# mikeoliphant/NeuralAudio

Hardware: AMD Instinct MI355X
Metric: concurrent 48 kHz real-time streams + Msamples/s/GPU, NAM WaveNet Standard (higher is better)
Workload: dtype f32 (f16x3-split MFMA, f32 accumulate)

## Files before the change

### neuralaudio_amd/csrc/wavenet_spec_impl.h

```cpp
#pragma once

#include <algorithm>
#include <atomic>
#include <cstddef>
#include <cstdlib>

#include <hip/hip_runtime.h>

#include "device_once.h"
#include <cstring>
#include <type_traits>
#include <vector>

#include "tuning.h"
#include "wavenet_split_dev.h"

namespace na
{
	namespace spk
	{
		using namespace sp;

#ifndef NA_SPK_NT_DIL
#define NA_SPK_NT_DIL 256
#endif
#ifndef NA_SPK_NT_LD
#define NA_SPK_NT_LD 0
#endif
#ifndef NA_SPK_NT_ST
#define NA_SPK_NT_ST 0
#endif
#ifndef NA_SPK_DELAY
#define NA_SPK_DELAY 0
#endif
#ifndef NA_SPK_AUX2
#define NA_SPK_AUX2 0
#endif
		typedef __attribute__((address_space(3))) char* LdsPtr;
		__device__ __forceinline__ u32x4 LdsRead16(unsigned addr) { return *reinterpret_cast<__attribute__((address_space(3))) const u32x4*>((LdsPtr)(size_t)addr); }
		__device__ __forceinline__ u32x2 LdsRead8(unsigned addr) { return *reinterpret_cast<__attribute__((address_space(3))) const u32x2*>((LdsPtr)(size_t)addr); }
		__device__ __forceinline__ void LdsWrite16(unsigned addr, u32x4 v) { *reinterpret_cast<__attribute__((address_space(3))) u32x4*>((LdsPtr)(size_t)addr) = v; }

		template <bool COH>
		__device__ __forceinline__ float LoadIn(const float* p)
		{
			if constexpr (COH) return __builtin_bit_cast(float, __hip_atomic_load(reinterpret_cast<const unsigned*>(p), __ATOMIC_RELAXED, __HIP_MEMORY_SCOPE_SYSTEM));
			else return *p;
		}
		template <bool COH>
		__device__ __forceinline__ void StoreOut(float* p, float v)
		{
			if constexpr (COH) __hip_atomic_store(reinterpret_cast<unsigned*>(p), __builtin_bit_cast(unsigned, v), __ATOMIC_RELAXED, __HIP_MEMORY_SCOPE_SYSTEM);
			else *p = v;
		}

		struct ArchA1Base
		{
			static constexpr int K(int, int) { return 3; }
			static constexpr int HEADK = 1;
			static constexpr bool LEAKY = false;
			static constexpr int T = 2, CHUNK = 10;
			static constexpr bool COARSE = false;
			static constexpr bool GUARDHIST = false;
			static constexpr bool FOLD = false;
			static constexpr int SKEW = 0;
			static constexpr bool COMPACT = true;
#ifndef NA_A1_NT_DIL
#define NA_A1_NT_DIL 128
#endif
			static constexpr int NT_DIL = NA_A1_NT_DIL;
		};
#ifndef NA_SPK_SKEW
#define NA_SPK_SKEW 0
#endif
		struct ArchStd : ArchA1Base
		{
			static constexpr int SKEW = NA_SPK_SKEW;
			static constexpr bool FOLD = true;
			static constexpr int NA = 2;
			static constexpr int CH[2] = { 16, 8 };
			static constexpr int NLA[2] = { 10, 10 };
			static constexpr int DIL[2][16] = { { 1, 2, 4, 8, 16, 32, 64, 128, 256, 512 }, { 1, 2, 4, 8, 16, 32, 64, 128, 256, 512 } };
		};
		struct ArchLite : ArchA1Base
		{
			static constexpr int NA = 2;
			static constexpr int CH[2] = { 16, 8 };
			static constexpr int NLA[2] = { 7, 13 };
			static constexpr int DIL[2][16] = { { 1, 2, 4, 8, 16, 32, 64 }, { 128, 256, 512, 1, 2, 4, 8, 16, 32, 64, 128, 256, 512 } };
		};
		struct ArchLite16 : ArchA1Base
		{
			static constexpr int NA = 2;
			static constexpr int CH[2] = { 16, 16 };
			static constexpr int NLA[2] = { 7, 13 };
			static constexpr int DIL[2][16] = { { 1, 2, 4, 8, 16, 32, 64 }, { 128, 256, 512, 1, 2, 4, 8, 16, 32, 64, 128, 256, 512 } };
		};

		struct ArchLite16T1 : ArchLite16 { static constexpr int T = 1; };

		struct ArchA2Base
		{
			static constexpr int NA = 1;
			static constexpr int NLA[2] = { 23, 0 };
			static constexpr int DIL[2][32] = { { 1, 3, 7, 17, 41, 101, 239, 1, 3, 7, 17, 41, 101, 239, 1, 13, 1, 3, 7, 17, 41, 101, 239 }, { 0 } };
			static constexpr int K(int, int l) { return (l == 14 || l == 15) ? 15 : 6; }
			static constexpr int HEADK = 16;
			static constexpr bool LEAKY = true;
			static constexpr int CHUNK = 16;
			static constexpr bool COARSE = true;
			static constexpr bool GUARDHIST = true;
			static constexpr bool FOLD = false;
			static constexpr int SKEW = 0;
			static constexpr bool COMPACT = false;
			static constexpr int NT_DIL = 100;
		};
		struct ArchA2Full : ArchA2Base { static constexpr int CH[2] = { 8, 0 }; static constexpr int T = 2; };
		struct ArchA2Lite : ArchA2Base { static constexpr int CH[2] = { 4, 0 }; static constexpr int T = 4; };

		struct FamStd { typedef ArchStd A0; typedef ArchStd A1; static constexpr int N = 1; };
		struct FamLite { typedef ArchLite A0; typedef ArchLite A1; static constexpr int N = 1; };
		struct FamLitePacked { typedef ArchLite A0; typedef ArchLite16 A1; static constexpr int N = 2; };
		struct FamA2 { typedef ArchA2Full A0; typedef ArchA2Lite A1; static constexpr int N = 2; };
		struct FamLite16T1 { typedef ArchLite16T1 A0; typedef ArchLite16T1 A1; static constexpr int N = 1; };

		enum TapClass { TAP_LDS = 0, TAP_HIST = 1, TAP_BOTH = 2 };

		template <class A>
		struct Tab
		{
			static constexpr int NA = A::NA;
			static constexpr int TotalLayers() { int n = 0; for (int a = 0; a < NA; a++) n += A::NLA[a]; return n; }
			static constexpr int NL = TotalLayers();
			static constexpr int NSTAGES = NL + NA + 1;
			static constexpr int ArrOf(int L) { int a = 0; while (L >= A::NLA[a]) { L -= A::NLA[a]; a++; } return a; }
			static constexpr int InArr(int L) { int a = 0; while (L >= A::NLA[a]) { L -= A::NLA[a]; a++; } return L; }
			static constexpr int Dil(int L) { return A::DIL[ArrOf(L)][InArr(L)]; }
			static constexpr int GPof(int a) { return A::CH[a] / 4; }
			static constexpr bool FirstOfArr(int L) { return InArr(L) == 0; }
			static constexpr bool LastOfArr(int L) { return InArr(L) == A::NLA[ArrOf(L)] - 1; }
			static constexpr int KS(int L) { return A::K(ArrOf(L), InArr(L)); }
			static constexpr bool Fold(int L) { return A::FOLD && KS(L) == 3 && GPof(ArrOf(L)) >= 2; }
			static constexpr int HEADK = A::HEADK;
			static constexpr int NRINGS = NL + (HEADK > 1 ? 1 : 0);
			static constexpr bool ExactRing(int L) { return L < NL && !FirstOfArr(L) && Dil(L) >= FRAMES && (KS(L) - 1) * Dil(L) >= 2 * FRAMES && ((KS(L) - 1) * Dil(L)) % 16 == 0; }
			static constexpr int HistFrames(int L) { return L < NL ? ((KS(L) - 1) * Dil(L) + 15) / 16 * 16 : (HEADK - 1 + 15) / 16 * 16; }
			static constexpr bool CompactRing(int L) { return A::COMPACT && L < NL && KS(L) > 1 && HistFrames(L) <= WN_COMPACT_MAX_HISTORY; }
			static constexpr int RingFrames(int L)
			{
				if (ExactRing(L)) return (KS(L) - 1) * Dil(L);
				if (CompactRing(L)) return 3 * HistFrames(L);
				return HistFrames(L) + FRAMES;
			}
			static constexpr int RingKeep(int L) { return ExactRing(L) ? RingFrames(L) : (CompactRing(L) ? HistFrames(L) : RingFrames(L) - FRAMES); }
			static constexpr int RingG(int L) { return GPof(L < NL ? ArrOf(L) : NA - 1); }
			static constexpr int RingOff(int L)
			{
				int o = WN_HEADER_F4;
				for (int l = 0; l < L; l++) o += RingFrames(l) * RingG(l);
				return o;
			}
			static constexpr int StateF4 = (RingOff(NRINGS) + 15) / 16 * 16;
			static constexpr int StageOfLayer(int L) { return 1 + L + ArrOf(L); }
			static constexpr int FirstLayerOfArr(int a) { int L = 0; for (int i = 0; i < a; i++) L += A::NLA[i]; return L; }
			static constexpr int LinkStage(int a) { return FirstLayerOfArr(a) + a; }
			static constexpr int LinkNC(int a) { const int Po = 4 / GPof(a - 1), Pn = 4 / GPof(a); return Po > Pn ? Po : Pn; }
			static constexpr int LayerOfStage(int s)
			{
				for (int L = 0; L < NL; L++)
					if (StageOfLayer(L) == s) return L;
				return -1;
			}
			static constexpr int StageOps(int s)
			{
				if (s == 0) return 1;
				if (s == NSTAGES - 1) return 2 * HEADK + 1;
				for (int a = 1; a < NA; a++)
					if (s == LinkStage(a)) return 4 * LinkNC(a) + 1;
				return 2 * KS(LayerOfStage(s)) + 4;
			}
			static constexpr int AOff(int s) { int o = 0; for (int i = 0; i < s; i++) o += StageOps(i) * 64; return o; }
			static constexpr int WsplitQuads = AOff(NSTAGES);
			static constexpr int CHUNK = A::CHUNK;
			static constexpr int TapOps(int s) { return s == NSTAGES - 1 ? 2 * HEADK : 2 * KS(LayerOfStage(s)); }
			static constexpr bool Chunked(int s) { return StageOps(s) > CHUNK; }
			static constexpr int TapChunks(int s) { return (TapOps(s) + CHUNK - 1) / CHUNK; }
			static constexpr int NumChunks(int s) { return Chunked(s) ? TapChunks(s) + 1 : 1; }
			static constexpr int ChunkBegin(int s, int c)
			{
				if (!Chunked(s)) return 0;
				if (c >= TapChunks(s)) return TapOps(s);
				const int pairs = TapOps(s) / 2, n = TapChunks(s);
				return 2 * ((pairs * c + n - 1) / n);
			}
			static constexpr int ChunkEnd(int s, int c) { return !Chunked(s) ? StageOps(s) : (c >= TapChunks(s) ? StageOps(s) : ChunkBegin(s, c + 1)); }
			static constexpr int ChunkIndex(int s, int c) { int n = 0; for (int i = 0; i < s; i++) n += NumChunks(i); return n + c; }
			static constexpr int MaxChunkOps()
			{
				int m = 0;
				for (int s = 0; s < NSTAGES; s++)
					for (int c = 0; c < NumChunks(s); c++) m = (ChunkEnd(s, c) - ChunkBegin(s, c)) > m ? (ChunkEnd(s, c) - ChunkBegin(s, c)) : m;
				return m;
			}
			static constexpr int MaxGP() { int m = 0; for (int a = 0; a < NA; a++) m = GPof(a) > m ? GPof(a) : m; return m; }
		};

		template <class A_, int NF_, int SPB_, bool PK_, bool COH_ = false, bool NT_ = false>
		struct Cfg
		{
			static constexpr bool COH = COH_;
			static constexpr bool NT = NT_;
			typedef A_ A;
			typedef Tab<A_> TB;
			static constexpr int NF = NF_, T = A_::T, FW = 16 * T, WPS = NF_ / FW, SPB = SPB_ * T / 2, NTHREADS = 64 * WPS * SPB;
			static_assert(WPS >= 1 && WPS * FW == NF_, "block length is a whole number of waves");
			static constexpr bool PK = PK_;
			static constexpr int MAXOPS = A_::CHUNK;
			static_assert(TB::MaxChunkOps() <= MAXOPS, "stage operand chunk");
			static constexpr int HPF = 5;
			static constexpr int SKEW = (SPB == 2 && !PK_ && T == 2 && A_::SKEW > 0) ? A_::SKEW : 0;
			static constexpr int NWB = SKEW > 0 ? SPB : 1;
			static constexpr int STG_THREADS = NTHREADS / NWB;
			static constexpr bool AUX16 = !PK_ && SKEW == 0;
			static constexpr int AUX_OFF = 0;
			static constexpr int IMG_OFF = AUX_OFF + SPB * FRAMES * (PK_ ? 32 : (AUX16 ? 16 : 8));
			static constexpr int IMG_ONE = TB::MaxGP() * PLANE * 16;
			static constexpr int WBUF_OFF = IMG_OFF + SPB * 2 * IMG_ONE;
			static constexpr int WBUF_ONE = MAXOPS * 1024;
			static constexpr int IDOP_OFF = WBUF_OFF + NWB * 2 * WBUF_ONE;
			static constexpr int DUMP_OFF = IDOP_OFF + 1024;
			static constexpr int FLAG_OFF = DUMP_OFF + 1024;
			static constexpr int BCAST_OFF = FLAG_OFF + 16 * SPB;
			static constexpr int LDS_BYTES = BCAST_OFF + (COH_ ? 64 : 0);
			static_assert(LDS_BYTES <= 80 * 1024, "two workgroups per CU");
		};

		template <int GP, int T>
		struct Geo
		{
			static_assert(GP == 4 || GP == 2 || GP == 1, "full lane modes of 16 / 8 / 4 channels");
			static constexpr int P = 4 / GP;
			static_assert(T % P == 0, "every tile slot of a set is a tile of the wave");
			static constexpr int S = T / P;
		};

		constexpr int TapClassOf(int F0, int P, int i, int shift)
		{
			const int lo = F0 + 16 * P * i - shift, hi = lo + 16 * P - 1;
			return hi < 0 ? TAP_HIST : (lo >= 0 ? TAP_LDS : TAP_BOTH);
		}

		template <class C, int RG>
		constexpr bool SmallRing() { return C::A::GUARDHIST && C::TB::RingKeep(RG) <= GUARD; }

		template <class C>
		constexpr int WaveTapClass(int w, int P, int i, int shift, bool small)
		{
			if (small) return TAP_LDS;
			if (!C::A::COARSE || w == 0 || C::WPS <= 2) return TapClassOf(C::FW * w, P, i, shift);
			const int first = TapClassOf(C::FW * 1, P, i, shift);
			for (int v = 2; v < C::WPS; v++)
				if (TapClassOf(C::FW * v, P, i, shift) != first) return TAP_BOTH;
			return first;
		}

		template <class C, int L>
		struct LayerSig
		{
			typedef typename C::TB TB;
			static constexpr int GP = TB::GPof(TB::ArrOf(L)), P = Geo<GP, C::T>::P, S = Geo<GP, C::T>::S, d = TB::Dil(L), K = TB::KS(L);
			static constexpr bool NEXT = !TB::LastOfArr(L);
			static constexpr int LN = NEXT ? L + 1 : L;
			static constexpr int dn = NEXT ? TB::Dil(LN) : 0, Kn = NEXT ? TB::KS(LN) : 1;
			static constexpr bool FOLD = TB::Fold(L) && !C::PK;
			static constexpr unsigned long long Of(int w)
			{
				unsigned long long s = 0;
				for (int k = 0; k < K - 1; k++)
					for (int i = 0; i < S; i++) s = s * 3 + (unsigned)WaveTapClass<C>(w, P, i, d * (K - 1 - k), SmallRing<C, L>());
				for (int k = 0; k < Kn - 1 && k < C::HPF; k++)
					for (int i = 0; i < S; i++) s = s * 3 + (unsigned)WaveTapClass<C>(w, P, i, dn * (Kn - 1 - k), SmallRing<C, LN>());
				return s;
			}
			static constexpr int Rep(int w) { int r = w; for (int v = w - 1; v >= 0; v--) if (Of(v) == Of(w)) r = v; return r; }
			static constexpr unsigned MaskOf(int r) { unsigned m = 0; for (int w = 0; w < C::WPS; w++) if (Rep(w) == r) m |= 1u << w; return m; }
			static constexpr bool LastRep(int r) { for (int w = r + 1; w < C::WPS; w++) if (Rep(w) == w) return false; return true; }
		};

		struct Ctx
		{
			__amdgpu_buffer_rsrc_t srsrc;
			__amdgpu_buffer_rsrc_t wrsrc;
			int myPos;
			int wave, sub, waveAll;
			int lane;
			int gs0, gs1;
			unsigned wbuf;
			int stgWave;
#ifdef NA_SP_TRACE
			long long* trace;
			int nwaves;
#endif
		};

#ifdef NA_SP_TRACE
#define SPK_STAMP(stage, point) do { __builtin_amdgcn_sched_barrier(0); if (cx.trace != nullptr && cx.lane == 0) cx.trace[(((stage) * 8 + (point)) * cx.nwaves) + cx.waveAll] = (long long)__builtin_readcyclecounter(); __builtin_amdgcn_sched_barrier(0); } while (0)
#else
#define SPK_STAMP(stage, point) (void)0
#endif

		template <class C, int GP>
		struct Lanes
// ... 127 lines not shown
			return (C::NF - C::FW) + 16 * P * (i + 1) - 1 >= C::NF - KEEP;
		}
		template <class C, int RG>
		constexpr int StoresOf()
		{
			constexpr int S = Geo<C::TB::RingG(RG), C::T>::S;
			int n = 0;
			for (int i = 0; i < S; i++) n += StoreNeeded<C, RG>(i) ? 1 : 0;
			return n;
		}

		template <class C, int RG, int GP, int MINSHIFT>
		__device__ __forceinline__ void Publish(const Ctx& cx, const Lanes<C, GP>& ln, u32x4 v, int i, int imgWrite)
		{
			typedef typename C::TB TB;
			constexpr int P = Geo<GP, C::T>::P, R = TB::RingFrames(RG), OFF = TB::RingOff(RG), KEEP = TB::RingKeep(RG);
			static_assert(GP == TB::RingG(RG), "lane mode of the receiving ring");
			if (!(NA_ABL & 64) && MINSHIFT < C::NF)
				LdsWrite16(ln.img + (unsigned)(imgWrite * C::IMG_ONE + 16 * P * i * 16), v);
			if ((NA_ABL & 4) || !StoreNeeded<C, RG>(i)) return;
			const int pos0 = __builtin_amdgcn_readlane(cx.myPos, RG);
			int base;
			if constexpr (TB::CompactRing(RG))
			{
				int end = pos0 + C::NF % R;
				if (end >= R) end -= R;
				base = end - C::NF + C::FW * cx.wave + 16 * P * i + R;
			}
			else
			{
				base = pos0 + C::FW * cx.wave + 16 * P * i;
				if (base >= R) base -= R;
			}
			const int addr = RingWrap<GP, R>(ln.ring, base);
			constexpr int NT_ST = C::NT ? 2 : NA_SPK_NT_ST, NT_DIL = C::NT ? C::A::NT_DIL : NA_SPK_NT_DIL;
			constexpr bool LONG = RG < TB::NL && TB::Dil(RG < TB::NL ? RG : 0) >= NT_DIL;
			if constexpr (LONG && NT_ST != 0)
			{
				if (KEEP >= C::NF) RingStoreAux<NT_ST>(cx.srsrc, v, addr, OFF * 16);
				else RingStoreAux<NT_ST>(cx.srsrc, v, (C::FW * cx.wave + 16 * P * i + ln.fl >= C::NF - KEEP) ? addr : OOB, OFF * 16);
				return;
			}
			if (KEEP >= C::NF) RingStore(cx.srsrc, v, addr, OFF * 16);
			else RingStore(cx.srsrc, v, (C::FW * cx.wave + 16 * P * i + ln.fl >= C::NF - KEEP) ? addr : OOB, OFF * 16);
		}

		template <class C, int RG, int GP>
		__device__ __forceinline__ void GuardStage(const Ctx& cx, const Lanes<C, GP>& ln, int imgBuf)
		{
			typedef typename C::TB TB;
			static_assert(GP == TB::RingG(RG), "lane mode of the ring");
			constexpr int R = TB::RingFrames(RG), OFF = TB::RingOff(RG);
			if constexpr (!C::A::GUARDHIST) return;
			if (cx.wave != 0) return;
			if constexpr (SmallRing<C, RG>())
			{
				if (NA_ABL & 4) return;
				const int pos0 = __builtin_amdgcn_readlane(cx.myPos, RG);
				int base = pos0 - GUARD;
				if (base < 0) base += R;
				if (cx.lane < 16)
				{
#pragma unroll
					for (int cg = 0; cg < GP; cg++)
					{
						const int addr = RingWrap<GP, R>((unsigned)((cx.lane * GP + cg) * 16), base);
						const unsigned dst = (unsigned)(C::IMG_OFF + imgBuf * C::IMG_ONE + cg * PLANE * 16) + (unsigned)(cx.sub * 2 * C::IMG_ONE);
						__builtin_amdgcn_raw_ptr_buffer_load_lds(cx.srsrc, (__attribute__((address_space(3))) void*)(LdsPtr)(size_t)dst, 16, addr, OFF * 16, 0, 0);
					}
				}
			}
			else
			{
				if ((cx.lane >> 4) < GP && (cx.lane & 15) == 15) LdsWrite16(ln.img + (unsigned)(imgBuf * C::IMG_ONE) - 16u * 16u, u32x4{ 0, 0, 0, 0 });
			}
		}

		template <class C, int SN, int CN>
		struct Stager
		{
			typedef typename C::TB TB;
			static constexpr int QUADS = (TB::ChunkEnd(SN, CN) - TB::ChunkBegin(SN, CN)) * 64;
			static constexpr int SRC = TB::AOff(SN) + TB::ChunkBegin(SN, CN) * 64;
			static constexpr int BUF = TB::ChunkIndex(SN, CN) & 1;
			static constexpr int NCOPY = (QUADS + C::STG_THREADS - 1) / C::STG_THREADS;
			static __device__ __forceinline__ void Begin(const Ctx& cx)
			{
				if (NA_ABL & 16) return;
#pragma unroll
				for (int c = 0; c < NCOPY; c++)
				{
					const int i0 = c * C::STG_THREADS + cx.stgWave * 64;
					const bool mine = i0 < QUADS;
					const unsigned dst = mine ? cx.wbuf + (unsigned)(BUF * C::WBUF_ONE) + (unsigned)i0 * 16u : (unsigned)C::DUMP_OFF;
					__builtin_amdgcn_raw_ptr_buffer_load_lds(cx.wrsrc, (__attribute__((address_space(3))) void*)(LdsPtr)(size_t)dst, 16,
						mine ? (SRC + i0 + cx.lane) * 16 : OOB, 0, 0, 0);
				}
			}
			template <int LATER>
			static __device__ __forceinline__ void End()
			{
				__builtin_amdgcn_s_waitcnt((LATER & 15) | ((LATER >> 4) << 14) | (7 << 4) | (15 << 8));
			}
		};
		template <class C, int s, int c>
		struct NextChunk
		{
			static constexpr bool SAME = c + 1 < C::TB::NumChunks(s);
			static constexpr int S = SAME ? s : s + 1, CN = SAME ? c + 1 : 0;
			typedef Stager<C, S, CN> St;
		};

		template <class C>
		__device__ __forceinline__ u32x4 WOp(const Ctx& cx, int s, int c, int m)
		{
			const int buf = C::TB::ChunkIndex(s, c) & 1, local = m - C::TB::ChunkBegin(s, c);
			return LdsRead16(cx.wbuf + (unsigned)(buf * C::WBUF_ONE + ((NA_ABL & 128) ? 0 : local) * 1024) + (unsigned)cx.lane * 16u);
		}

		template <bool PACKED>
		__device__ __forceinline__ f32x4 ActivateTanh(f32x4 a)
		{
			if (PACKED)
			{
				const f32x2 lo = FastTanh2(f32x2{ a.x, a.y }), hi = FastTanh2(f32x2{ a.z, a.w });
				return f32x4{ lo.x, lo.y, hi.x, hi.y };
			}
			return f32x4{ FastTanh(a.x), FastTanh(a.y), FastTanh(a.z), FastTanh(a.w) };
		}

		template <class C, int GP>
		__device__ __forceinline__ u32x4 TapLds(const Ctx& cx, const Lanes<C, GP>& ln, int imgRead, int shift, int i, int cls)
		{
			constexpr int P = Geo<GP, C::T>::P;
			if (NA_ABL & 256) return u32x4{ (unsigned)shift, 0, 0, 0 };
			if (cls == TAP_LDS) return LdsRead16(ln.img + (unsigned)(imgRead * C::IMG_ONE) + (unsigned)((16 * P * i - shift) * 16));
			int off = C::FW * cx.wave + 16 * P * i + ln.fl - shift;
			off = off < -1 ? -1 : off;
			return LdsRead16((unsigned)(C::IMG_OFF + imgRead * C::IMG_ONE + GUARD * 16) + (unsigned)(cx.sub * 2 * C::IMG_ONE) + (unsigned)((ln.cg * PLANE + off) * 16));
		}

		template <class C, int RG, int GP, int WR>
		__device__ __forceinline__ f32x4 ConvTap(const Ctx& cx, const Lanes<C, GP>& ln, int imgRead, int shift, int i, u32x4 ah, u32x4 al, u32x4 hist, f32x4 acc)
		{
			constexpr int P = Geo<GP, C::T>::P;
			const int cls = WaveTapClass<C>(WR, P, i, shift, SmallRing<C, RG>());
			if (cls != TAP_LDS)
			{
				acc = Mfma(ah, hist, acc);
				acc = MfmaLo<1>(al, hist, acc);
			}
			if (cls != TAP_HIST)
			{
				const u32x4 b = TapLds<C, GP>(cx, ln, imgRead, shift, i, cls);
				acc = Mfma(ah, b, acc);
				acc = MfmaLo<1>(al, b, acc);
			}
			return acc;
		}

		template <class C, int RG, int GP, int WR>
		__device__ __forceinline__ f32x4 ConvTapFold(const Ctx& cx, const Lanes<C, GP>& ln, int imgRead, int shift, int i, u32x4 ah, u32x4 hist, f32x4 acc, u32x2& th)
		{
			constexpr int P = Geo<GP, C::T>::P;
			const int cls = WaveTapClass<C>(WR, P, i, shift, SmallRing<C, RG>());
			th = u32x2{ 0, 0 };
			if (cls != TAP_LDS)
			{
				acc = Mfma(ah, hist, acc);
				th = u32x2{ hist.x, hist.y };
			}
			if (cls != TAP_HIST)
			{
				const u32x4 b = TapLds<C, GP>(cx, ln, imgRead, shift, i, cls);
				acc = Mfma(ah, b, acc);
				th = cls == TAP_LDS ? u32x2{ b.x, b.y } : u32x2{ th.x | b.x, th.y | b.y };
			}
			return acc;
		}

		template <class C, int L, int WR, int c>
		__device__ __forceinline__ void LayerChunk(const Ctx& cx, const Lanes<C, C::TB::GPof(C::TB::ArrOf(L))>& ln, State& st, u32x4 (&ax)[LayerSig<C, L>::S],
			f32x4 (&acc)[LayerSig<C, L>::S])
		{
			typedef typename C::TB TB;
			typedef LayerSig<C, L> SG;
			constexpr int GP = SG::GP, S = SG::S, K = SG::K, s = TB::StageOfLayer(L), NCH = TB::NumChunks(s), CB = TB::ChunkBegin(s, c), CE = TB::ChunkEnd(s, c);
			constexpr int imgRead = s & 1, imgWrite = (s + 1) & 1, LN = SG::LN;
			constexpr bool LASTLAYER = TB::LastOfArr(L) && TB::ArrOf(L) == TB::NA - 1;
			constexpr int NEXTMINSHIFT = SG::NEXT ? TB::Dil(LN) : (1 << 20);
			constexpr bool OWN = 2 * (K - 1) >= CB && 2 * (K - 1) < CE;
			constexpr bool TAIL = 2 * K >= CB && 2 * K < CE;
			constexpr int LATER = ((OWN && SG::NEXT) ? HistLoadsOf<C, LN>() : 0) + ((TAIL && SG::NEXT && !LASTLAYER) ? StoresOf<C, LN>() : 0);
			typedef typename NextChunk<C, s, c>::St NextStager;
			if constexpr (c == 0)
			{
				if constexpr (SG::NEXT) GuardStage<C, LN, GP>(cx, ln, imgWrite);
				else if constexpr (LASTLAYER && TB::HEADK > 1) GuardStage<C, TB::NL, GP>(cx, ln, (TB::NSTAGES - 1 + 1) & 1);
			}
			NextStager::Begin(cx);
			if constexpr (c == 0)
			{
#pragma unroll
				for (int i = 0; i < S; i++) ax[i] = AuxRead<C, GP>(ln, i);
			}
			constexpr int KLO = CB / 2, KHI = (CE / 2 < K - 1) ? CE / 2 : K - 1;
			constexpr int NX = (KHI > C::HPF) ? KHI - (KLO > C::HPF ? KLO : C::HPF) : 0;
			u32x4 hx[NX > 0 ? NX : 1][S];
#pragma unroll
			for (int k = KLO; k < KHI; k++)
			{
				if (k < C::HPF) continue;
#pragma unroll
				for (int i = 0; i < S; i++)
					if (WaveTapClass<C>(WR, SG::P, i, ShiftOf<C, L>(k), SmallRing<C, L>()) != TAP_LDS) hx[k - (KLO > C::HPF ? KLO : C::HPF)][i] = HistLoadAt<C, L, WR>(cx, ln.ring, ln.fl, ShiftOf<C, L>(k), i);
			}
			static_assert(!SG::FOLD || (NCH == 1 && K == 3), "folded operands: K = 3 layers in one chunk");
			u32x2 th[SG::FOLD ? 2 : 1][S];
#pragma unroll
			for (int k = KLO; k < KHI; k++)
			{
				const u32x4 ah = WOp<C>(cx, s, c, 2 * k), al = SG::FOLD ? ah : WOp<C>(cx, s, c, 2 * k + 1);
#pragma unroll
				for (int i = 0; i < S; i++)
				{
					u32x4 h = u32x4{ 0, 0, 0, 0 };
					if (WaveTapClass<C>(WR, SG::P, i, ShiftOf<C, L>(k), SmallRing<C, L>()) != TAP_LDS)
						h = (k < C::HPF) ? st.hist[k < C::HPF ? k : 0][i] : hx[k >= C::HPF ? k - (KLO > C::HPF ? KLO : C::HPF) : 0][i];
					if constexpr (SG::FOLD) acc[i] = ConvTapFold<C, L, GP, WR>(cx, ln, imgRead, ShiftOf<C, L>(k), i, ah, h, acc[i], th[k < 2 ? k : 0][i]);
					else acc[i] = ConvTap<C, L, GP, WR>(cx, ln, imgRead, ShiftOf<C, L>(k), i, ah, al, h, acc[i]);
				}
			}
			if constexpr (SG::FOLD)
			{
				const u32x4 al01 = WOp<C>(cx, s, c, 1);
#pragma unroll
				for (int i = 0; i < S; i++) acc[i] = Mfma(al01, u32x4{ th[0][i].x, th[0][i].y, th[1][i].x, th[1][i].y }, acc[i]);
			}
			if constexpr (OWN)
			{
				if constexpr (SG::NEXT) HistPrefetch<C, LN, WR>(cx, ln.ring, ln.fl, st);
				const u32x4 ah = WOp<C>(cx, s, c, 2 * K - 2), al = WOp<C>(cx, s, c, 2 * K - 1);
#pragma unroll
				for (int i = 0; i < S; i++)
				{
					acc[i] = Mfma(ah, st.xs[i], acc[i]);
					if constexpr (SG::FOLD) acc[i] = Mfma(al, u32x4{ st.xs[i].x, st.xs[i].y, ax[i].x, ax[i].y }, acc[i]);
					else acc[i] = MfmaLo<1>(al, st.xs[i], acc[i]);
				}
			}
			if constexpr (TAIL)
			{
				if constexpr (!SG::FOLD)
				{
					const u32x4 xa = WOp<C>(cx, s, c, 2 * K);
#pragma unroll
					for (int i = 0; i < S; i++) acc[i] = Mfma(xa, ax[i], acc[i]);
				}
				SPK_STAMP(s, 1);
				f32x4 z[S];
#pragma unroll
				for (int i = 0; i < S; i++)
				{
					if constexpr (C::A::LEAKY) z[i] = f32x4{ LeakyReLU(acc[i].x), LeakyReLU(acc[i].y), LeakyReLU(acc[i].z), LeakyReLU(acc[i].w) };
					else z[i] = ActivateTanh<(NA_PK_TANH != 0) && (C::NTHREADS < 512)>(acc[i]);
				}
				SPK_STAMP(s, 2);
				const u32x4 idop = LdsRead16((unsigned)C::IDOP_OFF + (unsigned)cx.lane * 16u);
				const u32x4 w1h = WOp<C>(cx, s, c, 2 * K + 1), w1l = WOp<C>(cx, s, c, 2 * K + 2), b1a = SG::FOLD ? w1l : WOp<C>(cx, s, c, 2 * K + 3);
#pragma unroll
				for (int i = 0; i < S; i++)
				{
					const u32x4 zs = SplitQuad(z[i]);
					st.hd[i] = Mfma(idop, zs, st.hd[i]);
					if constexpr (!LASTLAYER)
					{
						f32x4 y = st.xc[i];
						y = Mfma(w1h, zs, y);
						const u32x4 axi = NA_SPK_AUX2 ? AuxRead<C, GP>(ln, i) : ax[i];
						if constexpr (SG::FOLD) y = Mfma(w1l, u32x4{ zs.x, zs.y, axi.x, axi.y }, y);
						else
						{
							y = MfmaLo<2>(w1l, zs, y);
							y = Mfma(b1a, axi, y);
						}
						st.xc[i] = y;
						if constexpr (SG::NEXT)
						{
							st.xs[i] = Split<C>(y, cx);
							Publish<C, LN, GP, NEXTMINSHIFT>(cx, ln, st.xs[i], i, imgWrite);
						}
					}
				}
				SPK_STAMP(s, 3);
			}
			NextStager::template End<LATER>();
			SPK_STAMP(s, 4);
			BlockBarrier<C::NTHREADS / 64>();
			if constexpr (c + 1 < NCH) LayerChunk<C, L, WR, c + 1>(cx, ln, st, ax, acc);
		}

		template <class C, int L, int WR>
		__device__ __forceinline__ void LayerBody(const Ctx& cx, const Lanes<C, C::TB::GPof(C::TB::ArrOf(L))>& ln, State& st)
		{
			constexpr int S = LayerSig<C, L>::S;
			SPK_STAMP(C::TB::StageOfLayer(L), 0);
			u32x4 ax[S];
			f32x4 acc[S];
#pragma unroll
			for (int i = 0; i < S; i++) acc[i] = f32x4{ 0.0f, 0.0f, 0.0f, 0.0f };
			LayerChunk<C, L, WR, 0>(cx, ln, st, ax, acc);
			SPK_STAMP(C::TB::StageOfLayer(L), 5);
		}

		template <class C, int L, int W>
		__device__ __forceinline__ void LayerDispatch(const Ctx& cx, const Lanes<C, C::TB::GPof(C::TB::ArrOf(L))>& ln, State& st)
		{
			typedef LayerSig<C, L> SG;
			if constexpr (W < C::WPS)
			{
				if constexpr (SG::Rep(W) != W) LayerDispatch<C, L, W + 1>(cx, ln, st);
				else if constexpr (SG::LastRep(W)) LayerBody<C, L, W>(cx, ln, st);
				else
				{
					constexpr unsigned MASK = SG::MaskOf(W);
					if ((MASK >> cx.wave) & 1u) LayerBody<C, L, W>(cx, ln, st);
					else LayerDispatch<C, L, W + 1>(cx, ln, st);
				}
			}
		}

		template <class C, int L, int W>
		__device__ __forceinline__ void FirstHistDispatch(const Ctx& cx, unsigned laneRing, int fl, State& st)
		{
			typedef typename C::TB TB;
			constexpr int GP = TB::GPof(TB::ArrOf(L)), P = Geo<GP, C::T>::P, S = Geo<GP, C::T>::S;
			if constexpr (W < C::WPS)
			{
				constexpr bool same = [] {
					bool r = true;
					for (int w = W + 1; w < C::WPS; w++)
						for (int k = 0; k < PrefetchTaps<C, L>(); k++)
							for (int i = 0; i < S; i++) r = r && WaveTapClass<C>(w, P, i, ShiftOf<C, L>(k), SmallRing<C, L>()) == WaveTapClass<C>(W, P, i, ShiftOf<C, L>(k), SmallRing<C, L>());
					return r;
				}();
				if constexpr (same) HistPrefetch<C, L, W>(cx, laneRing, fl, st);
				else
				{
					if (cx.wave == W) HistPrefetch<C, L, W>(cx, laneRing, fl, st);
					else FirstHistDispatch<C, L, W + 1>(cx, laneRing, fl, st);
				}
			}
		}

		template <class C>
		__device__ __forceinline__ void RechStage(const Ctx& cx, const Lanes<C, C::TB::GPof(0)>& ln, State& st)
		{
			constexpr int GP = C::TB::GPof(0), S = Geo<GP, C::T>::S;
			SPK_STAMP(0, 0);
			GuardStage<C, 0, GP>(cx, ln, 1);
			const u32x4 ra = WOp<C>(cx, 0, 0, 0);
#pragma unroll
			for (int i = 0; i < S; i++)
			{
				const u32x4 ax = AuxRead<C, GP>(ln, i);
				f32x4 x = f32x4{ 0.0f, 0.0f, 0.0f, 0.0f };
				x = Mfma(ra, ax, x);
				st.xc[i] = x;
				st.hd[i] = f32x4{ 0.0f, 0.0f, 0.0f, 0.0f };
				st.xs[i] = Split<C>(x, cx);
				Publish<C, 0, GP, C::TB::Dil(0)>(cx, ln, st.xs[i], i, 1);
			}
			FirstHistDispatch<C, 0, 0>(cx, ln.ring, ln.fl, st);
			SPK_STAMP(0, 1); SPK_STAMP(0, 2); SPK_STAMP(0, 3);
			Stager<C, 1, 0>::template End<StoresOf<C, 0>() + HistLoadsOf<C, 0>()>();
			SPK_STAMP(0, 4);
			BlockBarrier<C::NTHREADS / 64>();
			SPK_STAMP(0, 5);
		}

		template <class C, int AN>
		__device__ __forceinline__ void LinkStage(const Ctx& cx, const Lanes<C, C::TB::GPof(AN)>& ln, State& st)
		{
			typedef typename C::TB TB;
			constexpr int GPO = TB::GPof(AN - 1), GPN = TB::GPof(AN), Po = 4 / GPO, Pn = 4 / GPN, NC = Po > Pn ? Po : Pn;
			constexpr int So = Geo<GPO, C::T>::S, Sn = Geo<GPN, C::T>::S, s = TB::LinkStage(AN), LN = TB::FirstLayerOfArr(AN);
			static_assert(C::T == 1 || C::T == 2, "array links are written for one or two tiles per wave");
			SPK_STAMP(s, 0);
			GuardStage<C, LN, GPN>(cx, ln, (s + 1) & 1);
			Stager<C, s + 1, 0>::Begin(cx);
			u32x4 hs[So], xq[So];
#pragma unroll
			for (int i = 0; i < So; i++)
			{
				hs[i] = Split<C>(st.hd[i], cx);
				xq[i] = Split<C>(st.xc[i], cx);
			}
			f32x4 hn[Sn], xn[Sn];
#pragma unroll
			for (int i = 0; i < Sn; i++)
			{
				hn[i] = f32x4{ 0.0f, 0.0f, 0.0f, 0.0f };
				xn[i] = f32x4{ 0.0f, 0.0f, 0.0f, 0.0f };
				hn[i] = Mfma(WOp<C>(cx, s, 0, 4 * NC), AuxRead<C, GPN>(ln, i), hn[i]);
			}
#pragma unroll
			for (int t = 0; t < C::T; t++)
			{
				const int u = t % NC, so = t / Po, sn = t / Pn;
hn[sn] = Mfma(WOp<C>(cx, s, 0, 4 * u), hs[so], hn[sn]);
				hn[sn] = MfmaLo<4>(WOp<C>(cx, s, 0, 4 * u + 1), hs[so], hn[sn]);
				xn[sn] = Mfma(WOp<C>(cx, s, 0, 4 * u + 2), xq[so], xn[sn]);
				xn[sn] = MfmaLo<4>(WOp<C>(cx, s, 0, 4 * u + 3), xq[so], xn[sn]);
			}
#pragma unroll
			for (int i = 0; i < Sn; i++)
			{
				st.hd[i] = hn[i];
				st.xc[i] = xn[i];
				st.xs[i] = Split<C>(xn[i], cx);
				Publish<C, LN, GPN, TB::Dil(LN)>(cx, ln, st.xs[i], i, (s + 1) & 1);
			}
			FirstHistDispatch<C, LN, 0>(cx, ln.ring, ln.fl, st);
			SPK_STAMP(s, 1); SPK_STAMP(s, 2); SPK_STAMP(s, 3);
			Stager<C, s + 1, 0>::template End<StoresOf<C, LN>() + HistLoadsOf<C, LN>()>();
			SPK_STAMP(s, 4);
			BlockBarrier<C::NTHREADS / 64>();
			SPK_STAMP(s, 5);
		}

		template <class C, int WR>
		__device__ __forceinline__ void HeadBody(const Ctx& cx, const Lanes<C, C::TB::GPof(C::TB::NA - 1)>& ln, State& st, float* __restrict__ out, size_t outBase,
			const long (&outRow)[4], int pack, float headScale, bool live)
		{
			typedef typename C::TB TB;
			constexpr int GP = TB::GPof(TB::NA - 1), P = Geo<GP, C::T>::P, S = Geo<GP, C::T>::S, s = TB::NSTAGES - 1, K = TB::HEADK, NCH = TB::NumChunks(s), RG = TB::NL;
			constexpr int imgHead = (s + 1) & 1;
			u32x4 hs[S];
			f32x4 acc[S];
#pragma unroll
			for (int i = 0; i < S; i++)
			{
				hs[i] = Split<C>(st.hd[i], cx);
				acc[i] = f32x4{ 0.0f, 0.0f, 0.0f, 0.0f };
			}
#pragma unroll
			for (int c = 0; c < NCH; c++)
			{
				if constexpr (K > 1)
				{
					if (c + 1 < NCH)
					{
						if (c == 0) Stager<C, s, 1>::Begin(cx);
						else if (c + 1 < NCH) Stager<C, s, (NCH > 2 ? 2 : 1)>::Begin(cx);
					}
					if (c == 0)
					{
#pragma unroll
						for (int i = 0; i < S; i++) Publish<C, RG, GP, 1>(cx, ln, hs[i], i, imgHead);
						BlockBarrier<C::NTHREADS / 64>();
					}
#pragma unroll
					for (int k = 0; k < K - 1; k++)
					{
						if (2 * k < TB::ChunkBegin(s, c) || 2 * k >= TB::ChunkEnd(s, c)) continue;
						const u32x4 ah = WOp<C>(cx, s, c, 2 * k), al = WOp<C>(cx, s, c, 2 * k + 1);
#pragma unroll
						for (int i = 0; i < S; i++)
						{
							u32x4 h = u32x4{ 0, 0, 0, 0 };
							if (WaveTapClass<C>(WR, P, i, K - 1 - k, SmallRing<C, RG>()) != TAP_LDS) h = HistLoadAt<C, RG, WR>(cx, ln.ring, ln.fl, K - 1 - k, i);
							acc[i] = ConvTap<C, RG, GP, WR>(cx, ln, imgHead, K - 1 - k, i, ah, al, h, acc[i]);
						}
					}
				}
				if (2 * (K - 1) >= TB::ChunkBegin(s, c) && 2 * (K - 1) < TB::ChunkEnd(s, c))
				{
					const u32x4 ah = WOp<C>(cx, s, c, 2 * K - 2), al = WOp<C>(cx, s, c, 2 * K - 1);
#pragma unroll
					for (int i = 0; i < S; i++)
					{
						acc[i] = Mfma(ah, hs[i], acc[i]);
						acc[i] = MfmaLo<8>(al, hs[i], acc[i]);
					}
				}
				if (2 * K >= TB::ChunkBegin(s, c) && 2 * K < TB::ChunkEnd(s, c))
				{
					const u32x4 ba = WOp<C>(cx, s, c, 2 * K);
#pragma unroll
					for (int i = 0; i < S; i++)
					{
						acc[i] = Mfma(ba, AuxRead<C, GP>(ln, i), acc[i]);
						const int f = C::FW * cx.wave + 16 * P * i + ln.fl;
						if (live && ln.cg == 0)
						{
							if constexpr (C::PK)
							{
								const float v[4] = { acc[i].x, acc[i].y, acc[i].z, acc[i].w };
#pragma unroll
								for (int q = 0; q < 4; q++)
									if (q < pack && outRow[q] >= 0) StoreOut<C::COH>(out + outRow[q] + f, headScale * v[q]);
							}
							else StoreOut<C::COH>(out + outBase + f, headScale * acc[i].x);
						}
					}
				}
				if (c + 1 < NCH)
				{
					__builtin_amdgcn_s_waitcnt(0 | (7 << 4) | (15 << 8));
					BlockBarrier<C::NTHREADS / 64>();
				}
			}
		}

		template <class C>
		__device__ __forceinline__ void HeadDispatch(const Ctx& cx, const Lanes<C, C::TB::GPof(C::TB::NA - 1)>& ln, State& st, float* __restrict__ out, size_t outBase,
			const long (&outRow)[4], int pack, float headScale, bool live)
		{
			if constexpr (C::TB::HEADK == 1 || C::WPS == 1 || SmallRing<C, C::TB::NL>()) HeadBody<C, 0>(cx, ln, st, out, outBase, outRow, pack, headScale, live);
			else
			{
				if (cx.wave == 0) HeadBody<C, 0>(cx, ln, st, out, outBase, outRow, pack, headScale, live);
				else HeadBody<C, C::WPS - 1>(cx, ln, st, out, outBase, outRow, pack, headScale, live);
			}
		}

		template <class C, int L, int LEND>
		__device__ __forceinline__ void RunLayers(const Ctx& cx, const Lanes<C, C::TB::GPof(C::TB::ArrOf(L))>& ln, State& st)
		{
			LayerDispatch<C, L, 0>(cx, ln, st);
			if constexpr (L + 1 < LEND) RunLayers<C, L + 1, LEND>(cx, ln, st);
		}

		template <class C, int AN>
		__device__ __forceinline__ void RunArrays(const Ctx& cx, State& st, float* __restrict__ out, size_t outBase, const long (&outRow)[4], int pack, float headScale, bool live)
		{
			typedef typename C::TB TB;
			Lanes<C, TB::GPof(AN)> ln;
			ln.Init(cx, AN == 0 ? cx.gs0 : cx.gs1);
			if constexpr (AN == 0) RechStage<C>(cx, ln, st);
			else LinkStage<C, AN>(cx, ln, st);
			RunLayers<C, TB::FirstLayerOfArr(AN), TB::FirstLayerOfArr(AN) + C::A::NLA[AN]>(cx, ln, st);
			if constexpr (AN + 1 < TB::NA) RunArrays<C, AN + 1>(cx, st, out, outBase, outRow, pack, headScale, live);
			else HeadDispatch<C>(cx, ln, st, out, outBase, outRow, pack, headScale, live);
		}

		template <class C>
		__device__ __forceinline__ void RunWorkgroup(const GroupArgs& ga, int groupBlock, const float* __restrict__ in, float* __restrict__ out, long inStride, long outStride
#ifdef NA_SP_TRACE
			, long long* trace
#endif
			, const int tid = (int)threadIdx.x
			)
		{
			typedef typename C::TB TB;
			constexpr bool PK = C::PK;
			constexpr int SPB = C::SPB, NF = C::NF;
			const int lane = tid & 63;
			const int waveAll = __builtin_amdgcn_readfirstlane(tid >> 6);
			const int sub = waveAll / C::WPS, wave = waveAll % C::WPS;

			int sidx = groupBlock * SPB + sub;
			const bool live = sidx < ga.numStreams;
			if (!live) sidx = ga.numStreams - 1;
			const int slot = ga.slots ? ga.slots[sidx] : ga.slot0 + sidx;
			const int row = PK ? 0 : (ga.slots ? ga.rows[sidx] : ga.row0 + sidx);
			u32x4* stt = ga.state + (size_t)slot * (size_t)ga.stateF4;
			int* header = reinterpret_cast<int*>(stt);

			Ctx cx;
			cx.srsrc = MakeRsrc(stt, live ? (unsigned)ga.stateF4 * 16u : 0u);
			cx.wrsrc = MakeRsrc(ga.wsplit, (unsigned)ga.wsplitQuads * 16u);
			cx.myPos = header[lane];
			cx.wave = wave; cx.sub = sub; cx.waveAll = waveAll; cx.lane = lane;
			cx.wbuf = (unsigned)(C::WBUF_OFF + (C::SKEW > 0 ? sub : 0) * 2 * C::WBUF_ONE);
			cx.stgWave = C::SKEW > 0 ? wave : waveAll;
#ifdef NA_SP_TRACE
			cx.trace = trace;
			cx.nwaves = C::NTHREADS / 64;
			if (cx.trace != nullptr && lane == 0) cx.trace[((C::TB::NSTAGES * 8 + 0) * cx.nwaves) + waveAll] = (long long)__builtin_readcyclecounter();
#endif
			Stager<C, 1, 0>::Begin(cx);
			const int pack = PK ? ga.pack : 1;
			cx.gs0 = PK ? ((ga.gps0 >> 1) & 3) : 0;
			cx.gs1 = PK ? (ga.gps1 == 0 ? -1 : ((ga.gps1 >> 1) & 3)) : 0;
			long outRow[4];
			int rowOf[4];
#pragma unroll
			for (int q = 0; q < 4; q++)
			{
				const int r = (PK && live && q < ga.pack) ? ga.rows[sidx * ga.pack + q] : -1;
				rowOf[q] = r;
				outRow[q] = r >= 0 ? (long)r * outStride : -1;
			}

			if constexpr (PK)
			{
				for (int i = wave * 64 + lane; i < FRAMES; i += C::WPS * 64)
				{
					float c[4];
#pragma unroll
					for (int q = 0; q < 4; q++) c[q] = (rowOf[q] >= 0 && i < NF) ? LoadIn<C::COH>(in + (size_t)rowOf[q] * inStride + i) : 0.0f;
#pragma unroll
					for (int q = 0; q < 4; q++)
					{
						const float cc = ClampCond(c[q], ga.condLimit);
						const _Float16 ch = (_Float16)cc, cl = (_Float16)(cc - (float)ch);
						const f16x2 a = { ch, (_Float16)1.0f }, b = { cl, (_Float16)1.0f };
						*reinterpret_cast<__attribute__((address_space(3))) u32x2*>((LdsPtr)(size_t)(unsigned)(C::AUX_OFF + ((sub * 4 + q) * FRAMES + i) * 8)) =
							u32x2{ __builtin_bit_cast(unsigned, a), __builtin_bit_cast(unsigned, b) };
					}
				}
			}
			else
			{
				for (int i = wave * 64 + lane; i < FRAMES; i += C::WPS * 64)
				{
					const float c = (i < NF) ? ClampCond(LoadIn<C::COH>(in + (size_t)row * inStride + i), ga.condLimit) : 0.0f;
					const _Float16 ch = (_Float16)c, cl = (_Float16)(c - (float)ch);
					const f16x2 a = { ch, (_Float16)1.0f }, b = { cl, (_Float16)1.0f }, d = { ch, (_Float16)0.0f };
					if constexpr (C::AUX16)
						LdsWrite16((unsigned)(C::AUX_OFF + (sub * FRAMES + i) * 16), u32x4{ __builtin_bit_cast(unsigned, a), __builtin_bit_cast(unsigned, b), __builtin_bit_cast(unsigned, d), 0u });
					else
						*reinterpret_cast<__attribute__((address_space(3))) u32x2*>((LdsPtr)(size_t)(unsigned)(C::AUX_OFF + (sub * FRAMES + i) * 8)) =
							u32x2{ __builtin_bit_cast(unsigned, a), __builtin_bit_cast(unsigned, b) };
				}
			}
			for (int i = tid; i < SPB * 2 * TB::MaxGP(); i += C::NTHREADS) LdsWrite16((unsigned)(C::IMG_OFF + (i * PLANE + GUARD - 1) * 16), u32x4{ 0, 0, 0, 0 });
			if (tid < 64)
			{
				const int i = lane & 15, q = lane >> 4;
				const unsigned one = 0x3c00u;
				const unsigned lo = (q == (i >> 2)) ? (((i & 3) == 0) ? one : ((i & 3) == 1) ? (one << 16) : 0u) : 0u;
				const unsigned hi = (q == (i >> 2)) ? (((i & 3) == 2) ? one : ((i & 3) == 3) ? (one << 16) : 0u) : 0u;
				LdsWrite16((unsigned)C::IDOP_OFF + (unsigned)lane * 16u, u32x4{ lo, hi, lo, hi });
			}
			if constexpr (C::A::LEAKY)
			{
				if (tid < SPB) *reinterpret_cast<__attribute__((address_space(3))) unsigned*>((LdsPtr)(size_t)(unsigned)(C::FLAG_OFF + 16 * tid)) = 0u;
			}
			if (cx.stgWave == 0) LdsWrite16(cx.wbuf + (unsigned)lane * 16u, BufLoad(cx.wrsrc, lane * 16));
			BlockBarrier<C::NTHREADS / 64>();

			if constexpr (C::SKEW > 0)
			{
				if (sub != 0)
					for (int k = 0; k < C::SKEW; k++) BlockBarrier<C::NTHREADS / 64>();
			}
			State st;
			RunArrays<C, 0>(cx, st, out, (size_t)row * outStride, outRow, pack, ga.headScale, live);
			if constexpr (C::SKEW > 0)
			{
				if (sub == 0)
					for (int k = 0; k < C::SKEW; k++) BlockBarrier<C::NTHREADS / 64>();
			}

#ifdef NA_SP_TRACE
			if (cx.trace != nullptr && lane == 0) cx.trace[((C::TB::NSTAGES * 8 + 1) * cx.nwaves) + waveAll] = (long long)__builtin_readcyclecounter();
// ... 433 lines not shown
```

Measured before the change: 3680.

## Triple-buffer weight staging two stages ahead for the Standard WaveNet

Adds a configurable weight-staging depth and sets it to three for the Standard architecture. Each stage's weight DMA into LDS is now issued two stages ahead instead of one, and the vmcnt waits are recomputed to count the history loads, stores and ahead DMA still in flight. The full block barrier is also replaced with a lighter wait plus s_barrier, so weight loads get more time to land behind compute. The cost is one more LDS weight buffer, which may lower occupancy, and more intricate wait-count bookkeeping that would corrupt results if a count is wrong.

```diff
diff --git a/neuralaudio_amd/csrc/wavenet_spec_impl.h b/neuralaudio_amd/csrc/wavenet_spec_impl.h
--- a/neuralaudio_amd/csrc/wavenet_spec_impl.h
+++ b/neuralaudio_amd/csrc/wavenet_spec_impl.h
@@ -64,6 +64,7 @@
 			static constexpr bool GUARDHIST = false;
 			static constexpr bool FOLD = false;
 			static constexpr int SKEW = 0;
+			static constexpr int WDEPTH = 2;
 			static constexpr bool COMPACT = true;
 #ifndef NA_A1_NT_DIL
 #define NA_A1_NT_DIL 128
@@ -76,6 +77,7 @@
 		struct ArchStd : ArchA1Base
 		{
 			static constexpr int SKEW = NA_SPK_SKEW;
+			static constexpr int WDEPTH = 3;
 			static constexpr bool FOLD = true;
 			static constexpr int NA = 2;
 			static constexpr int CH[2] = { 16, 8 };
@@ -112,6 +114,7 @@
 			static constexpr bool GUARDHIST = true;
 			static constexpr bool FOLD = false;
 			static constexpr int SKEW = 0;
+			static constexpr int WDEPTH = 2;
 			static constexpr bool COMPACT = false;
 			static constexpr int NT_DIL = 100;
 		};
@@ -195,6 +198,7 @@
 			}
 			static constexpr int ChunkEnd(int s, int c) { return !Chunked(s) ? StageOps(s) : (c >= TapChunks(s) ? StageOps(s) : ChunkBegin(s, c + 1)); }
 			static constexpr int ChunkIndex(int s, int c) { int n = 0; for (int i = 0; i < s; i++) n += NumChunks(i); return n + c; }
+			static constexpr bool AnyChunked() { for (int s = 0; s < NSTAGES; s++) if (Chunked(s)) return true; return false; }
 			static constexpr int MaxChunkOps()
 			{
 				int m = 0;
@@ -221,13 +225,18 @@
 			static constexpr int SKEW = (SPB == 2 && !PK_ && T == 2 && A_::SKEW > 0) ? A_::SKEW : 0;
 			static constexpr int NWB = SKEW > 0 ? SPB : 1;
 			static constexpr int STG_THREADS = NTHREADS / NWB;
+			static constexpr int WDEPTH = A_::WDEPTH;
+			static_assert(WDEPTH == 2 || WDEPTH == 3, "staging depth");
+			static_assert(WDEPTH != 3 || SKEW == 0, "depth 3: the streams of a workgroup share one set of buffers");
+			static_assert(WDEPTH != 3 || !TB::AnyChunked(), "depth 3: every stage is one chunk");
+			static_assert(WDEPTH != 3 || !A_::GUARDHIST, "depth 3: no guard DMA among the counted VMEM operations");
 			static constexpr bool AUX16 = !PK_ && SKEW == 0;
 			static constexpr int AUX_OFF = 0;
 			static constexpr int IMG_OFF = AUX_OFF + SPB * FRAMES * (PK_ ? 32 : (AUX16 ? 16 : 8));
 			static constexpr int IMG_ONE = TB::MaxGP() * PLANE * 16;
 			static constexpr int WBUF_OFF = IMG_OFF + SPB * 2 * IMG_ONE;
 			static constexpr int WBUF_ONE = MAXOPS * 1024;
-			static constexpr int IDOP_OFF = WBUF_OFF + NWB * 2 * WBUF_ONE;
+			static constexpr int IDOP_OFF = WBUF_OFF + NWB * WDEPTH * WBUF_ONE;
 			static constexpr int DUMP_OFF = IDOP_OFF + 1024;
 			static constexpr int FLAG_OFF = DUMP_OFF + 1024;
 			static constexpr int BCAST_OFF = FLAG_OFF + 16 * SPB;
@@ -521,7 +530,7 @@
 			typedef typename C::TB TB;
 			static constexpr int QUADS = (TB::ChunkEnd(SN, CN) - TB::ChunkBegin(SN, CN)) * 64;
 			static constexpr int SRC = TB::AOff(SN) + TB::ChunkBegin(SN, CN) * 64;
-			static constexpr int BUF = TB::ChunkIndex(SN, CN) & 1;
+			static constexpr int BUF = TB::ChunkIndex(SN, CN) % C::WDEPTH;
 			static constexpr int NCOPY = (QUADS + C::STG_THREADS - 1) / C::STG_THREADS;
 			static __device__ __forceinline__ void Begin(const Ctx& cx)
 			{
@@ -539,6 +548,7 @@
 			template <int LATER>
 			static __device__ __forceinline__ void End()
 			{
+				static_assert(LATER >= 0 && LATER <= 63, "vmcnt is six bits");
 				__builtin_amdgcn_s_waitcnt((LATER & 15) | ((LATER >> 4) << 14) | (7 << 4) | (15 << 8));
 			}
 		};
@@ -550,10 +560,73 @@
 			typedef Stager<C, S, CN> St;
 		};
 
+		template <class C, int s>
+		constexpr int AheadStores()
+		{
+			typedef typename C::TB TB;
+			if constexpr (s < 0 || s >= TB::NSTAGES - 1) return 0;
+			else if constexpr (TB::LayerOfStage(s) < 0) return StoresOf<C, TB::LayerOfStage(s + 1)>();
+			else if constexpr (TB::LastOfArr(TB::LayerOfStage(s))) return 0;
+			else return StoresOf<C, TB::LayerOfStage(s) + 1>();
+		}
+		template <class C, int L, int WR>
+		constexpr int HistUsedBy()
+		{
+			typedef typename C::TB TB;
+			constexpr int GP = TB::GPof(TB::ArrOf(L)), P = Geo<GP, C::T>::P, S = Geo<GP, C::T>::S;
+			int n = 0;
+			for (int k = 0; k < PrefetchTaps<C, L>(); k++)
+				for (int i = 0; i < S; i++)
+					n += (HistNeededAt<C, GP>(ShiftOf<C, L>(k), i, SmallRing<C, L>()) && WaveTapClass<C>(WR, P, i, ShiftOf<C, L>(k), SmallRing<C, L>()) != TAP_LDS) ? 1 : 0;
+			return n;
+		}
+		template <class C, int s>
+		constexpr int AheadDma()
+		{
+			if constexpr (s < 0 || s + 2 >= C::TB::NSTAGES) return 0;
+			else return Stager<C, s + 2, 0>::NCOPY;
+		}
+		template <class C, int s>
+		constexpr int AheadTail()
+		{
+			if constexpr (s < 0) return 0;
+			else return C::TB::LayerOfStage(s) < 0 ? 0 : AheadStores<C, s>();
+		}
+		__device__ __forceinline__ void AheadFence() { __builtin_amdgcn_sched_barrier(0x1 | 0x2 | 0x4 | 0x8 | 0x80 | 0x100 | 0x200 | 0x400); }
+		template <class C, int s>
+		constexpr int AheadLater(int hist) { return AheadTail<C, s - 1>() + hist + AheadDma<C, s>() + AheadStores<C, s>(); }
+		template <class C, int SN, int HIST>
+		__device__ __forceinline__ void AheadClose(const Ctx& cx)
+		{
+			if constexpr (SN >= 0)
+			{
+				if constexpr (AheadDma<C, SN>() > 0)
+				{
+					if constexpr (HIST > 0) AheadFence();
+					Stager<C, SN + 2, 0>::Begin(cx);
+				}
+				Stager<C, SN + 1, 0>::template End<AheadLater<C, SN>(HIST)>();
+			}
+		}
+
+		template <class C>
+		__device__ __forceinline__ void StageBarrier()
+		{
+			if constexpr (C::WDEPTH == 3)
+			{
+				if (NA_ABL & 8) return;
+				__builtin_amdgcn_s_waitcnt(15 | (3 << 14) | (7 << 4) | (0 << 8));
+				asm volatile("" ::: "memory");
+				__builtin_amdgcn_s_barrier();
+				asm volatile("" ::: "memory");
+			}
+			else BlockBarrier<C::NTHREADS / 64>();
+		}
+
 		template <class C>
 		__device__ __forceinline__ u32x4 WOp(const Ctx& cx, int s, int c, int m)
 		{
-			const int buf = C::TB::ChunkIndex(s, c) & 1, local = m - C::TB::ChunkBegin(s, c);
+			const int buf = C::TB::ChunkIndex(s, c) % C::WDEPTH, local = m - C::TB::ChunkBegin(s, c);
 			return LdsRead16(cx.wbuf + (unsigned)(buf * C::WBUF_ONE + ((NA_ABL & 128) ? 0 : local) * 1024) + (unsigned)cx.lane * 16u);
 		}
 
@@ -630,14 +703,18 @@
 			constexpr int NEXTMINSHIFT = SG::NEXT ? TB::Dil(LN) : (1 << 20);
 			constexpr bool OWN = 2 * (K - 1) >= CB && 2 * (K - 1) < CE;
 			constexpr bool TAIL = 2 * K >= CB && 2 * K < CE;
-			constexpr int LATER = ((OWN && SG::NEXT) ? HistLoadsOf<C, LN>() : 0) + ((TAIL && SG::NEXT && !LASTLAYER) ? StoresOf<C, LN>() : 0);
+			constexpr bool AHEAD = C::WDEPTH == 3;
+			constexpr int LATER2 = ((OWN && SG::NEXT) ? HistLoadsOf<C, LN>() : 0) + ((TAIL && SG::NEXT && !LASTLAYER) ? StoresOf<C, LN>() : 0);
+			constexpr int LATER = AHEAD ? AheadLater<C, s>(SG::NEXT ? HistUsedBy<C, LN, WR>() : 0) : LATER2;
+			static_assert(!AHEAD || (NCH == 1 && K - 1 <= C::HPF), "depth 3: one chunk, every shifted tap's history prefetched");
 			typedef typename NextChunk<C, s, c>::St NextStager;
 			if constexpr (c == 0)
 			{
 				if constexpr (SG::NEXT) GuardStage<C, LN, GP>(cx, ln, imgWrite);
 				else if constexpr (LASTLAYER && TB::HEADK > 1) GuardStage<C, TB::NL, GP>(cx, ln, (TB::NSTAGES - 1 + 1) & 1);
 			}
-			NextStager::Begin(cx);
+			if constexpr (!AHEAD) NextStager::Begin(cx);
+			else if constexpr (!SG::NEXT && s + 2 < TB::NSTAGES) Stager<C, s + 2, 0>::Begin(cx);
 			if constexpr (c == 0)
 			{
 #pragma unroll
@@ -679,6 +756,11 @@
 			if constexpr (OWN)
 			{
 				if constexpr (SG::NEXT) HistPrefetch<C, LN, WR>(cx, ln.ring, ln.fl, st);
+				if constexpr (AHEAD && SG::NEXT)
+				{
+					AheadFence();
+					Stager<C, s + 2, 0>::Begin(cx);
+				}
 				const u32x4 ah = WOp<C>(cx, s, c, 2 * K - 2), al = WOp<C>(cx, s, c, 2 * K - 1);
 #pragma unroll
 				for (int i = 0; i < S; i++)
@@ -735,7 +817,7 @@
 			}
 			NextStager::template End<LATER>();
 			SPK_STAMP(s, 4);
-			BlockBarrier<C::NTHREADS / 64>();
+			StageBarrier<C>();
 			if constexpr (c + 1 < NCH) LayerChunk<C, L, WR, c + 1>(cx, ln, st, ax, acc);
 		}
 
@@ -769,7 +851,7 @@
 			}
 		}
 
-		template <class C, int L, int W>
+		template <class C, int L, int W, int SN = -1>
 		__device__ __forceinline__ void FirstHistDispatch(const Ctx& cx, unsigned laneRing, int fl, State& st)
 		{
 			typedef typename C::TB TB;
@@ -783,11 +865,19 @@
 							for (int i = 0; i < S; i++) r = r && WaveTapClass<C>(w, P, i, ShiftOf<C, L>(k), SmallRing<C, L>()) == WaveTapClass<C>(W, P, i, ShiftOf<C, L>(k), SmallRing<C, L>());
 					return r;
 				}();
-				if constexpr (same) HistPrefetch<C, L, W>(cx, laneRing, fl, st);
+				if constexpr (same)
+				{
+					HistPrefetch<C, L, W>(cx, laneRing, fl, st);
+					AheadClose<C, SN, HistUsedBy<C, L, W>()>(cx);
+				}
 				else
 				{
-					if (cx.wave == W) HistPrefetch<C, L, W>(cx, laneRing, fl, st);
-					else FirstHistDispatch<C, L, W + 1>(cx, laneRing, fl, st);
+					if (cx.wave == W)
+					{
+						HistPrefetch<C, L, W>(cx, laneRing, fl, st);
+						AheadClose<C, SN, HistUsedBy<C, L, W>()>(cx);
+					}
+					else FirstHistDispatch<C, L, W + 1, SN>(cx, laneRing, fl, st);
 				}
 			}
 		}
@@ -810,11 +900,19 @@
 				st.xs[i] = Split<C>(x, cx);
 				Publish<C, 0, GP, C::TB::Dil(0)>(cx, ln, st.xs[i], i, 1);
 			}
-			FirstHistDispatch<C, 0, 0>(cx, ln.ring, ln.fl, st);
-			SPK_STAMP(0, 1); SPK_STAMP(0, 2); SPK_STAMP(0, 3);
-			Stager<C, 1, 0>::template End<StoresOf<C, 0>() + HistLoadsOf<C, 0>()>();
+			if constexpr (C::WDEPTH == 3)
+			{
+				SPK_STAMP(0, 1); SPK_STAMP(0, 2); SPK_STAMP(0, 3);
+				FirstHistDispatch<C, 0, 0, 0>(cx, ln.ring, ln.fl, st);
+			}
+			else
+			{
+				FirstHistDispatch<C, 0, 0>(cx, ln.ring, ln.fl, st);
+				SPK_STAMP(0, 1); SPK_STAMP(0, 2); SPK_STAMP(0, 3);
+				Stager<C, 1, 0>::template End<StoresOf<C, 0>() + HistLoadsOf<C, 0>()>();
+			}
 			SPK_STAMP(0, 4);
-			BlockBarrier<C::NTHREADS / 64>();
+			StageBarrier<C>();
 			SPK_STAMP(0, 5);
 		}
 
@@ -827,7 +925,7 @@
 			static_assert(C::T == 1 || C::T == 2, "array links are written for one or two tiles per wave");
 			SPK_STAMP(s, 0);
 			GuardStage<C, LN, GPN>(cx, ln, (s + 1) & 1);
-			Stager<C, s + 1, 0>::Begin(cx);
+			if constexpr (C::WDEPTH == 2) Stager<C, s + 1, 0>::Begin(cx);
 			u32x4 hs[So], xq[So];
 #pragma unroll
 			for (int i = 0; i < So; i++)
@@ -860,11 +958,19 @@
 				st.xs[i] = Split<C>(xn[i], cx);
 				Publish<C, LN, GPN, TB::Dil(LN)>(cx, ln, st.xs[i], i, (s + 1) & 1);
 			}
-			FirstHistDispatch<C, LN, 0>(cx, ln.ring, ln.fl, st);
-			SPK_STAMP(s, 1); SPK_STAMP(s, 2); SPK_STAMP(s, 3);
-			Stager<C, s + 1, 0>::template End<StoresOf<C, LN>() + HistLoadsOf<C, LN>()>();
+			if constexpr (C::WDEPTH == 3)
+			{
+				SPK_STAMP(s, 1); SPK_STAMP(s, 2); SPK_STAMP(s, 3);
+				FirstHistDispatch<C, LN, 0, s>(cx, ln.ring, ln.fl, st);
+			}
+			else
+			{
+				FirstHistDispatch<C, LN, 0>(cx, ln.ring, ln.fl, st);
+				SPK_STAMP(s, 1); SPK_STAMP(s, 2); SPK_STAMP(s, 3);
+				Stager<C, s + 1, 0>::template End<StoresOf<C, LN>() + HistLoadsOf<C, LN>()>();
+			}
 			SPK_STAMP(s, 4);
-			BlockBarrier<C::NTHREADS / 64>();
+			StageBarrier<C>();
 			SPK_STAMP(s, 5);
 		}
 
@@ -875,6 +981,7 @@
 			typedef typename C::TB TB;
 			constexpr int GP = TB::GPof(TB::NA - 1), P = Geo<GP, C::T>::P, S = Geo<GP, C::T>::S, s = TB::NSTAGES - 1, K = TB::HEADK, NCH = TB::NumChunks(s), RG = TB::NL;
 			constexpr int imgHead = (s + 1) & 1;
+			static_assert(C::WDEPTH == 2 || NCH == 1, "depth 3: the head's operands were set out two stages ago and awaited by the last layer; nothing is left to stage");
 			u32x4 hs[S];
 			f32x4 acc[S];
 #pragma unroll
@@ -1012,7 +1119,7 @@
 			cx.wrsrc = MakeRsrc(ga.wsplit, (unsigned)ga.wsplitQuads * 16u);
 			cx.myPos = header[lane];
 			cx.wave = wave; cx.sub = sub; cx.waveAll = waveAll; cx.lane = lane;
-			cx.wbuf = (unsigned)(C::WBUF_OFF + (C::SKEW > 0 ? sub : 0) * 2 * C::WBUF_ONE);
+			cx.wbuf = (unsigned)(C::WBUF_OFF + (C::SKEW > 0 ? sub : 0) * C::WDEPTH * C::WBUF_ONE);
 			cx.stgWave = C::SKEW > 0 ? wave : waveAll;
 #ifdef NA_SP_TRACE
 			cx.trace = trace;
```

Measured after the change: 3755 (median of 4 runs). 2.0% higher.
